# wukailu/single-stable-dreamfusion

Measured on AMD Instinct MI355X. Metric: SDS train steps/sec + rays/sec at 128×128, 1/2/4/8 MI355X, higher is better.
Workload: dtype fp16+f32; 1 GPU; C2: -O (fp16, cuda_ray, dir_text) 128x128 render, batch 1, max_steps 512, density grid update every 16 steps; global_batch=1, parallelism=dp1, backward=fused, launch=hip-graph replay, grad_exchange=none (one rank), optimizer_in_graph=True

## Files before the change

include/dfhip.h:

```cpp
#ifndef DFHIP_H
#define DFHIP_H

#include <stdint.h>

#ifdef __cplusplus
extern "C" {
#endif

typedef void *dfhip_stream_t;

enum dfhip_dtype { DFHIP_F32 = 0, DFHIP_F16 = 1, DFHIP_F64 = 2, DFHIP_BF16 = 3 };
enum dfhip_shading {
    DFHIP_SHADING_ALBEDO = 0,
    DFHIP_SHADING_TEXTURELESS = 1,
    DFHIP_SHADING_LAMBERTIAN = 2,
    DFHIP_SHADING_NORMAL = 3
};

enum dfhip_status {
    DFHIP_OK = 0,
    DFHIP_EINVAL = 1,
    DFHIP_EDTYPE = 2,
    DFHIP_ELAUNCH = 3,
    DFHIP_ENOMEM = 4
// ... 403 lines not shown
                                         const float *grad_loss, float lambda, float *loss,
                                         dfhip_stream_t stream);
int dfhip_ray_head_forward_backward_entropy_loss(
    uint32_t N, const float *ws, const float *depth, const float *image, const float *rays_d,
    const float *nears, const float *fars, const float *w1, const float *b1, const float *w2,
    const float *b2, float *out_image, float *out_depth, uint8_t *mask, const float *g_image,
    float *grad_image, float *grad_ws, float *partial, float *gw1, float *gb1, float *gw2,
    float *gb2, const float *grad_loss, float lambda, float *loss, dfhip_stream_t stream);
int dfhip_ray_head_backward_check(uint32_t N, const float *g_image, const float *ws,
                                  const float *rays_d, const float *w1, const float *b1,
                                  const float *w2, const float *b2, const float *bg_color,
                                  float *grad_image, float *grad_ws, float *grad_bg,
                                  float *partial, float *gw1, float *gb1, float *gw2, float *gb2,
                                  const float *grad_loss, float lambda, float *loss,
                                  float *found_inf, dfhip_stream_t stream);
int dfhip_ray_head_forward_backward_entropy_loss_check(
    uint32_t N, const float *ws, const float *depth, const float *image, const float *rays_d,
    const float *nears, const float *fars, const float *w1, const float *b1, const float *w2,
    const float *b2, float *out_image, float *out_depth, uint8_t *mask, const float *g_image,
    float *grad_image, float *grad_ws, float *partial, float *gw1, float *gb1, float *gw2,
    float *gb2, const float *grad_loss, float lambda, float *loss, float *found_inf,
    int defer_sum, dfhip_stream_t stream);

int dfhip_entropy_forward(uint32_t N, const float *ws, float lambda, float *loss,
                          dfhip_stream_t stream);
int dfhip_entropy_backward(uint32_t N, const float *ws, const float *grad_loss, float lambda,
                           float *grad_ws, dfhip_stream_t stream);
int dfhip_entropy_backward_accumulate(uint32_t N, const float *ws, const float *grad_loss,
                                      float lambda, float *grad_ws, dfhip_stream_t stream);

int dfhip_train_step_prologue(const float *pose, float fx, float fy, float cx, float cy,
                              uint32_t H, uint32_t W, const float *aabb, float min_near,
                              uint64_t seed, uint64_t step, int perturb, const float *alphas,
                              uint32_t min_step, uint32_t max_step, float *rays_o,
                              float *rays_d, float *nears, float *fars, float *noises,
                              float *bg_color, float *g_image, int32_t *counter,
                              dfhip_stream_t stream);
int dfhip_train_step_prologue_lr(const float *pose, float fx, float fy, float cx, float cy,
                                 uint32_t H, uint32_t W, const float *aabb, float min_near,
                                 uint64_t seed, uint64_t step, int perturb, const float *alphas,
                                 uint32_t min_step, uint32_t max_step, float *rays_o,
                                 float *rays_d, float *nears, float *fars, float *noises,
                                 float *bg_color, float *g_image, int32_t *counter,
                                 const float *lr_host, uint32_t n_lr, float *lr_dev,
                                 dfhip_stream_t stream);
int dfhip_train_step_prologue_row(const float *pose, float fx, float fy, float cx, float cy,
// ... 128 lines not shown
```

single-stable-dreamfusion_amd/_dfhip.py:

```python
from __future__ import annotations

import ctypes
import os
from pathlib import Path

import torch

LIB_PATH = Path(os.environ.get("DFHIP_LIB", Path(__file__).resolve().parent / "lib" / "libdfhip.so"))

F32, F16, F64, BF16 = 0, 1, 2, 3
_DTYPE = {torch.float32: F32, torch.float16: F16, torch.float64: F64, torch.bfloat16: BF16}

_vp, _u32, _i32, _f32 = ctypes.c_void_p, ctypes.c_uint32, ctypes.c_int, ctypes.c_float
_u64 = ctypes.c_uint64

_SIGS = {
    "dfhip_near_far_from_aabb": [_i32, _vp, _vp, _vp, _u32, _f32, _vp, _vp, _vp],
    "dfhip_get_rays": [_vp, _f32, _f32, _f32, _f32, _u32, _u32, _vp, _vp, _vp],
    "dfhip_density_grid_ema": [_vp, _vp, _u32, _u32, _f32, _vp, _vp, _vp],
    "dfhip_packbits_mean": [_vp, _u32, _vp, _f32, _vp, _vp, _vp],
    "dfhip_mean_count": [_vp, _u32, _vp, _vp],
    "dfhip_sph_from_ray": [_i32, _vp, _vp, _f32, _u32, _vp, _vp],
    "dfhip_morton3D": [_vp, _u32, _vp, _vp],
    "dfhip_morton3D_invert": [_vp, _u32, _vp, _vp],
# ... 79 lines not shown
    "dfhip_grid_field_forward_quads": [_i32, _vp, _f32, _vp, _vp, _vp, _u32, _f32, _u32, _u32,
                                       _i32, _vp, _vp, _vp, _vp, _vp, _vp, _vp, _vp, _vp, _i32,
                                       _u32, _vp, _vp],
    "dfhip_grid_field_forward_bf16": [_vp, _f32, _vp, _vp, _u32, _f32, _u32, _u32, _i32, _vp,
                                      _vp, _vp, _vp, _vp, _vp, _vp, _vp, _vp, _i32, _u32, _vp,
                                      _vp],
    "dfhip_grid_field_backward_bf16": [_vp, _vp, _f32, _vp, _vp, _vp, _vp, _vp, _vp, _vp, _vp,
                                       _i32, _u32, _vp, _vp, _vp, _u32, _vp, _vp, _vp, _vp, _vp,
                                       _vp, _i32, _vp],
    "dfhip_grid_field_backward_accumulate": [
        _vp, _vp, _f32, _vp, _vp, _vp, _vp, _vp, _vp, _vp, _vp, _i32, _u32, _vp, _vp, _vp, _u32,
        _vp, _vp, _vp, _vp, _vp, _vp, _vp, _u32, _u32, _f32, _u32, _u32, _i32, _vp, _vp, _u32,
        _vp],
    "dfhip_adam_amp_step": [_i32, _vp, _vp, _vp, _vp, _vp, _vp, _vp, _vp, _vp, _vp, _vp, _vp,
                            _vp, _vp, _f32, _f32, _i32, _vp],
    "dfhip_adam_amp_step_lr_dev": [_i32, _vp, _vp, _vp, _vp, _vp, _vp, _vp, _vp, _vp, _vp, _vp,
                                   _vp, _vp, _vp, _vp, _f32, _f32, _i32, _vp],
    "dfhip_adam_amp_step_tail": [_i32, _vp, _vp, _vp, _vp, _vp, _vp, _vp, _vp, _vp, _vp, _vp,
                                 _vp, _vp, _vp, _vp, _f32, _f32, _i32, _u32, _vp, _vp, _vp, _vp],
    "dfhip_ray_head_backward_check": [_u32, _vp, _vp, _vp, _vp, _vp, _vp, _vp, _vp, _vp, _vp,
                                      _vp, _vp, _vp, _vp, _vp, _vp, _vp, _f32, _vp, _vp, _vp],
    "dfhip_ray_head_forward_backward_entropy_loss_check": [_u32] + [_vp] * 22 + [_f32, _vp, _vp,
                                                                                 _i32, _vp],
    "dfhip_param_grad_sums": [_vp, _u32, _vp, _vp, _vp, _vp, _vp, _vp, _i32, _u32, _vp, _vp, _vp,
                              _vp, _vp, _vp, _f32, _vp, _vp, _vp],
    "dfhip_grid_field_backward_check": [_i32, _vp, _vp, _f32, _vp, _vp, _vp, _vp, _vp, _vp, _vp,
                                        _vp, _i32, _u32, _vp, _vp, _vp, _u32, _vp, _vp, _vp, _vp,
                                        _vp, _vp, _i32, _vp, _i32, _vp],
    "dfhip_march_rays_train_count_staged_quads": [_i32, _vp, _vp, _vp, _f32, _f32, _u32, _u32,
                                                  _u32, _u32, _vp, _vp, _vp, _vp, _vp, _vp, _vp,
                                                  _i32, _vp, _vp, _u32, _f32, _u32, _u32, _i32,
                                                  _u32, _vp, _vp, _vp],
    "dfhip_train_step_prologue_row": [_vp, _f32, _f32, _f32, _f32, _u32, _u32, _vp, _f32,
                                      ctypes.c_uint64, ctypes.c_uint64, _i32, _vp, _u32, _u32,
                                      _vp, _vp, _vp, _vp, _vp, _vp, _vp, _vp, _vp, _u32, _vp,
                                      _u32, _vp, _vp],
    "dfhip_ray_head_forward": [_u32, _vp, _vp, _vp, _vp, _vp, _vp, _vp, _vp, _vp, _vp, _vp, _vp,
                               _vp, _vp, _vp],
    "dfhip_ray_head_backward": [_u32, _vp, _vp, _vp, _vp, _vp, _vp, _vp, _vp, _vp, _vp, _vp, _vp,
                                _vp, _vp, _vp, _vp, _vp],
    "dfhip_ray_head_backward_entropy": [_u32, _vp, _vp, _vp, _vp, _vp, _vp, _vp, _vp, _vp, _vp,
                                        _vp, _vp, _vp, _vp, _vp, _vp, _vp, _f32, _vp],
    "dfhip_ray_head_forward_backward_entropy_loss": [_u32] + [_vp] * 22 + [_f32, _vp, _vp],
    "dfhip_ray_head_backward_entropy_loss": [_u32, _vp, _vp, _vp, _vp, _vp, _vp, _vp, _vp, _vp,
                                             _vp, _vp, _vp, _vp, _vp, _vp, _vp, _vp, _f32, _vp,
                                             _vp],
# ... 228 lines not shown
```

single-stable-dreamfusion_amd/csrc/head.hip:

```cpp
#include "common.h"
#include "field_common.h"

#include <math.h>

namespace dfhip {
namespace hd {

constexpr int kDeg = 6;
constexpr int kIn = 3 + 3 * 2 * kDeg;
constexpr int kHid = 64;
constexpr int kOut = 3;
constexpr int kW1 = kHid * kIn, kB1 = kHid, kW2 = kOut * kHid, kB2 = kOut;
constexpr int kParams = kW1 + kB1 + kW2 + kB2;
constexpr float kHalfPi = 3.141592653589793f / 2.0f;

__device__ __forceinline__ float r16(float x) { return (float)(half_t)f32_rounded(x); }

struct alignas(16) W {
    float w1t[kW1], b1[kB1], w2[kW2], b2[kB2];
};

__device__ __forceinline__ void load_w(W &w, const float *w1, const float *b1, const float *w2,
                                       const float *b2) {
    for (int i = threadIdx.x; i < kW1; i += blockDim.x) {
// ... 150 lines not shown
#pragma unroll
    for (int k = 0; k < 3; ++k) {
        g[k] = g_image[(size_t)k * N + n];
        grad_image[3 * (size_t)n + k] = g[k];
        const float bg = bg_color ? bg_color[3 * (size_t)n + k] : 1.0f;
        sw = sw + g[k] * bg;
        if (grad_bg) grad_bg[3 * (size_t)n + k] = g[k] * t;
    }
    grad_ws[n] = -sw;
}

constexpr float kLo = 1e-5f, kHi = 1.0f - 1e-5f;

__device__ __forceinline__ float entropy_grad(uint32_t N, float a, const float *g, float lambda) {
    const float scale = g[0] * lambda / (float)N;
    return (a >= kLo && a <= kHi) ? scale * (log2f(1.0f - a) - log2f(a)) : 0.0f;
}

struct FwdIO {
    const float *depth, *image, *nears, *fars;
    float *out_image, *out_depth;
    uint8_t *mask;
};

template <bool FWD>
__global__ __launch_bounds__(kThreads) void k_head_bwd_net(
    uint32_t N, const float *__restrict__ g_image , const float *__restrict__ ws,
    const float *__restrict__ rays_d, const float *w1, const float *b1, const float *w2,
    const float *b2, float *__restrict__ grad_image, float *__restrict__ grad_ws,
    float *__restrict__ partial, const float *__restrict__ ent_grad_loss, float ent_lambda,
    FwdIO io) {
    __shared__ W w;
    __shared__ alignas(16) float s_x[kRays][kIn + 1];
    __shared__ half_t s_dh[kRays][kHid];
    __shared__ half_t s_h[kRays][kHid];
    __shared__ float s_do[kRays][4];
    load_w(w, w1, b1, w2, b2);
    const int q = threadIdx.x & (kSub - 1), r = threadIdx.x / kSub;
    const uint32_t n = blockIdx.x * kRays + r;
    const bool live = n < N;
    if (live) features_part(rays_d + 3 * (size_t)n, q, s_x[r]);
    else if (q == 0)
        for (int i = 0; i < kIn; ++i) s_x[r][i] = 0.0f;
    __syncthreads();
    float x[kIn], h[kPer], o[kOut];
    load_x(s_x[r], true, x);
// ... 24 lines not shown
        grad_ws[n] = ent_grad_loss ? -sw + entropy_grad(N, ws[n], ent_grad_loss, ent_lambda)
                                   : -sw;
    }
    const float t = live ? 1.0f - ws[n] : 0.0f;
    float dout[3];
#pragma unroll
    for (int k = 0; k < 3; ++k) {
        const float dbg = r16(g[k] * t);
        dout[k] = r16(dbg * (1.0f - bg[k]) * bg[k]);
    }
#pragma unroll
    for (int jj = 0; jj < kPer; ++jj) {
        const int j = kPer * q + jj;
        float a = 0.0f;
#pragma unroll
        for (int k = 0; k < kOut; ++k) a = fmaf(dout[k], w.w2[k * kHid + j], a);
        s_dh[r][j] = (half_t)(h[jj] > 0.0f ? r16(a) : 0.0f);
        s_h[r][j] = (half_t)h[jj];
    }
    if (q == 0)
#pragma unroll
        for (int k = 0; k < kOut; ++k) s_do[r][k] = dout[k];
    __syncthreads();
    float *out = partial + (size_t)blockIdx.x * kParams;
    for (int p = threadIdx.x; p < kParams; p += blockDim.x) {
        float s = 0.0f;
        if (p < kW1) {
            const int j = p / kIn, i = p - j * kIn;
            for (int y = 0; y < kRays; ++y) s = fmaf((float)s_dh[y][j], s_x[y][i], s);
        } else if (p < kW1 + kB1) {
            const int j = p - kW1;
            for (int y = 0; y < kRays; ++y) s += (float)s_dh[y][j];
        } else if (p < kW1 + kB1 + kW2) {
            const int k = (p - kW1 - kB1) / kHid, j = (p - kW1 - kB1) - k * kHid;
            for (int y = 0; y < kRays; ++y) s = fmaf(s_do[y][k], (float)s_h[y][j], s);
        } else {
            const int k = p - kW1 - kB1 - kW2;
            for (int y = 0; y < kRays; ++y) s += s_do[y][k];
        }
        out[p] = s;
    }
}

__device__ __forceinline__ void entropy_loss_block(uint32_t N, const float *__restrict__ ws,
                                                   float lambda, float *__restrict__ loss);

__device__ __forceinline__ void wsum_block(uint32_t blk, const float *__restrict__ partial,
                                           uint32_t blocks, float *gw1, float *gb1, float *gw2,
                                           float *gb2, float *found_inf) {
    __shared__ float red[16][64];
    const int o = threadIdx.x & 63, grp = threadIdx.x >> 6;
    const int p = blk * 64 + o;
    float s = 0.0f;
    if (p < kParams) {
        uint32_t b = grp;
        for (; b + 7 * 16 < blocks; b += 8 * 16) {
            float x[8];
#pragma unroll
            for (int u = 0; u < 8; ++u) x[u] = partial[(size_t)(b + 16 * u) * kParams + p];
#pragma unroll
            for (int u = 0; u < 8; ++u) s += x[u];
        }
        for (; b < blocks; b += 16) s += partial[(size_t)b * kParams + p];
    }
    red[grp][o] = s;
// ... 281 lines not shown
    float *grad_image, float *grad_ws, float *partial, float *gw1, float *gb1, float *gw2,
    float *gb2, const float *grad_loss, float lambda, float *loss, float *found_inf,
    int defer_sum, dfhip_stream_t stream) {
    const char *name = "ray_head_forward_backward_entropy_loss_check";
    if (!loss) {
        set_error("%s: null loss", name);
        return DFHIP_EINVAL;
    }
    if (N == 0) {
        set_error("%s: N must be > 0", name);
        return DFHIP_EINVAL;
    }
    if (!w1 || !depth || !image || !nears || !fars || !out_image || !out_depth || !mask ||
        !grad_loss) {
        set_error("%s: null pointer (the combined launch needs the background network)", name);
        return DFHIP_EINVAL;
    }
    const hd::FwdIO io{depth, image, nears, fars, out_image, out_depth, mask};
    return ray_head_backward(N, g_image, ws, rays_d, w1, b1, w2, b2, nullptr, grad_image,
                             grad_ws, nullptr, partial, gw1, gb1, gw2, gb2, grad_loss, lambda,
                             stream, loss, &io, found_inf, defer_sum != 0);
}

extern "C" int dfhip_param_grad_sums(const float *mlp_partial, uint32_t mlp_parts, float *gw1,
                                     float *gb1, float *gw2, float *gb2, float *gw3, float *gb3,
                                     int accumulate, uint32_t N, const float *head_partial,
                                     float *hgw1, float *hgb1, float *hgw2, float *hgb2,
                                     const float *ws, float lambda, float *loss,
                                     float *found_inf, dfhip_stream_t stream) {
    const char *name = "param_grad_sums";
    if (!mlp_partial || mlp_parts == 0 || !gw1 || !gb1 || !gw2 || !gb2 || !gw3 || !gb3) {
        set_error("%s: null pointer or no parts in the field role", name);
        return DFHIP_EINVAL;
    }
    if (head_partial && (N == 0 || !hgw1 || !hgb1 || !hgw2 || !hgb2)) {
        set_error("%s: the head role needs N > 0 and its four gradients", name);
        return DFHIP_EINVAL;
    }
    if ((ws != nullptr) != (loss != nullptr)) {
        set_error("%s: the entropy role needs both ws and loss", name);
        return DFHIP_EINVAL;
    }
    const hd::FieldSum f{mlp_partial, mlp_parts, gw1, gb1, gw2, gb2, gw3, gb3, accumulate};
    const hd::HeadSum h{head_partial, ceil_div(N, (uint32_t)hd::kRays), hgw1, hgb1, hgw2, hgb2,
                        ws, N, lambda, loss};
    const uint32_t blocks = hd::kFieldSumBlocks + (head_partial ? hd::kHeadSumBlocks : 0u) +
// ... 40 lines not shown
```

single-stable-dreamfusion_amd/csrc/raymarching.hip:

```cpp
#include "field_common.h"
#include "march_common.h"

#include <type_traits>

namespace dfhip {
namespace rm {


template <typename T> __device__ __forceinline__ T max_value();
template <> __device__ __forceinline__ float max_value<float>() { return FLT_MAX; }
template <> __device__ __forceinline__ double max_value<double>() { return DBL_MAX; }
template <> __device__ __forceinline__ half_t max_value<half_t>() { return (half_t)65504.0f; }

template <typename scalar_t>
__global__ __launch_bounds__(256) void k_near_far(const scalar_t *__restrict__ rays_o,
                                                  const scalar_t *__restrict__ rays_d,
                                                  const scalar_t *__restrict__ aabb,
                                                  uint32_t N, float min_near,
                                                  scalar_t *nears, scalar_t *fars) {
    const uint32_t n = blockIdx.x * blockDim.x + threadIdx.x;
    if (n >= N) return;
    const Ray r = load_ray(rays_o + 3 * n, rays_d + 3 * n);
    float b[6];
#pragma unroll
// ... 280 lines not shown
    acc_t T = 1, r = 0, g = 0, b = 0, ws = 0, t = 0, d = 0;
    if (num != 0 && offset + num <= M) {
        const scalar_t *s = sigmas + offset;
        const rgb_t *c = rgbs + 3 * (size_t)offset;
        const scalar_t *dl = deltas + 2 * (size_t)offset;
        for (uint32_t i = 0; i < num; ++i) {
            const acc_t alpha = (acc_t)1.0f - (acc_t)__expf(-to_f(s[i]) * to_f(dl[2 * i]));
            const acc_t w = alpha * T;
            r = fma(w, (acc_t)to_f(c[3 * i + 0]), r);
            g = fma(w, (acc_t)to_f(c[3 * i + 1]), g);
            b = fma(w, (acc_t)to_f(c[3 * i + 2]), b);
            t += (acc_t)to_f(dl[2 * i + 1]);
            d = fma(w, t, d);
            ws += w;
            T *= (acc_t)1.0f - alpha;
            if (T < (acc_t)T_thresh) break;
        }
    }
    weights_sum[index] = (scalar_t)ws;
    depth[index] = (scalar_t)d;
    image[3 * index + 0] = (scalar_t)r;
    image[3 * index + 1] = (scalar_t)g;
    image[3 * index + 2] = (scalar_t)b;
}

template <typename scalar_t, typename rgb_t, typename acc_t>
__device__ __forceinline__ rgb_t grad_cast(acc_t v) { return (rgb_t)v; }
template <>
__device__ __forceinline__ half_t grad_cast<float, half_t, float>(float v) {
    return (half_t)f32_rounded(v);
}
template <>
__device__ __forceinline__ bf16_t grad_cast<float, bf16_t, float>(float v) {
    return (bf16_t)f32_rounded(v);
}

template <typename scalar_t, bool DENSE, typename rgb_t = scalar_t>
__global__ __launch_bounds__(64) void k_composite_train_bwd(
    const scalar_t *__restrict__ grad_ws, const scalar_t *__restrict__ grad_image,
    const scalar_t *__restrict__ sigmas, const rgb_t *__restrict__ rgbs,
    const scalar_t *__restrict__ deltas, const int32_t *__restrict__ rays,
    const scalar_t *__restrict__ weights_sum, const scalar_t *__restrict__ image,
    uint32_t M, uint32_t N, float T_thresh, scalar_t *grad_sigmas, rgb_t *grad_rgbs,
    int tail = 1) {
    typedef typename Acc<scalar_t>::type acc_t;
    const uint32_t n = blockIdx.x * 64 + threadIdx.x;
    if (n >= N) return;
    const uint32_t index = (uint32_t)rays[3 * n];
    const uint32_t offset = (uint32_t)rays[3 * n + 1];
    const uint32_t num = (uint32_t)rays[3 * n + 2];
    const scalar_t zero = (scalar_t)0.0f;
    const rgb_t czero = (rgb_t)0.0f;
    uint32_t i = 0;
    if (num != 0 && offset + num <= M) {
        const scalar_t *s = sigmas + offset;
        const rgb_t *c = rgbs + 3 * (size_t)offset;
        const scalar_t *dl = deltas + 2 * (size_t)offset;
// ... 25 lines not shown
            acc = fma(gb, fma(T, cb, -(bf - b)), acc);
            acc = fma(gw, (acc_t)1 - wsf, acc);
            gs[i] = (scalar_t)(dt * acc);
            if (T < (acc_t)T_thresh) { ++i; break; }
        }
    }
    if (DENSE) {
        const uint64_t end = min((uint64_t)offset + num, (uint64_t)M);
        for (uint64_t row = (uint64_t)offset + i; row < end; ++row) {
            grad_sigmas[row] = zero;
            grad_rgbs[3 * row] = czero; grad_rgbs[3 * row + 1] = czero; grad_rgbs[3 * row + 2] = czero;
        }
        if (tail && n == N - 1) {
            for (uint64_t row = (uint64_t)offset + num; row < M; ++row) {
                grad_sigmas[row] = zero;
                grad_rgbs[3 * row] = czero; grad_rgbs[3 * row + 1] = czero; grad_rgbs[3 * row + 2] = czero;
            }
        }
    }
}

constexpr uint32_t kCompRaysPerBlock = 16;

template <int J>
__device__ __forceinline__ float row_bcast(float v) {
    return __int_as_float(
        __builtin_amdgcn_update_dpp(0, __float_as_int(v), 0x150 + J, 0xF, 0xF, false));
}

template <typename rgb_t>
__device__ __forceinline__ void load_rgb3(const rgb_t *c, float &r, float &g, float &b) {
    r = to_f(c[0]);
    g = to_f(c[1]);
    b = to_f(c[2]);
}

struct FwdChain {
    float T = 1.0f, r = 0.0f, g = 0.0f, b = 0.0f, ws = 0.0f, t = 0.0f, d = 0.0f;
    bool alive = true;
    template <int J>
    __device__ __forceinline__ void step(float a, float om, float cr, float cg, float cb,
                                         float dl, float T_thresh) {
        const float w = alive ? row_bcast<J>(a) * T : 0.0f;
        r = fmaf(w, row_bcast<J>(cr), r);
        g = fmaf(w, row_bcast<J>(cg), g);
        b = fmaf(w, row_bcast<J>(cb), b);
        t += row_bcast<J>(dl);
        d = fmaf(w, t, d);
        ws += w;
        T *= row_bcast<J>(om);
        alive = alive && !(T < T_thresh);
    }
};

template <typename scalar_t, typename rgb_t>
__global__ __launch_bounds__(256) void k_composite_train_fwd_w(
    const scalar_t *__restrict__ sigmas, const rgb_t *__restrict__ rgbs,
    const scalar_t *__restrict__ deltas, const int32_t *__restrict__ rays, uint32_t M,
    uint32_t N, float T_thresh, scalar_t *weights_sum, scalar_t *depth, scalar_t *image) {
    const uint32_t n = blockIdx.x * kCompRaysPerBlock + (threadIdx.x >> 4);
    const int lane = (int)(threadIdx.x & 15);
    uint32_t index = 0, offset = 0, num = 0;
    if (n < N) {
        index = (uint32_t)rays[3 * n];
        offset = (uint32_t)rays[3 * n + 1];
        num = (uint32_t)rays[3 * n + 2];
        if (offset + num > M) num = 0;
    }
    FwdChain c;
    for (uint32_t base = 0; base < num && c.alive; base += 16) {
        const uint32_t cnt = min(16u, num - base);
        float a = 0.0f, om = 1.0f, cr = 0.0f, cg = 0.0f, cb = 0.0f, dl = 0.0f;
        if ((uint32_t)lane < cnt) {
            const size_t i = (size_t)offset + base + lane;
            a = 1.0f - __expf(-to_f(sigmas[i]) * to_f(deltas[2 * i]));
            om = 1.0f - a;
            dl = to_f(deltas[2 * i + 1]);
            load_rgb3(rgbs + 3 * i, cr, cg, cb);
        }
#define DFHIP_FSTEP(J) c.step<J>(a, om, cr, cg, cb, dl, T_thresh);
        DFHIP_FSTEP(0) DFHIP_FSTEP(1) DFHIP_FSTEP(2) DFHIP_FSTEP(3)
        DFHIP_FSTEP(4) DFHIP_FSTEP(5) DFHIP_FSTEP(6) DFHIP_FSTEP(7)
        DFHIP_FSTEP(8) DFHIP_FSTEP(9) DFHIP_FSTEP(10) DFHIP_FSTEP(11)
        DFHIP_FSTEP(12) DFHIP_FSTEP(13) DFHIP_FSTEP(14) DFHIP_FSTEP(15)
#undef DFHIP_FSTEP
    }
    if (lane == 0 && n < N) {
        weights_sum[index] = (scalar_t)c.ws;
        depth[index] = (scalar_t)c.d;
        image[3 * index + 0] = (scalar_t)c.r;
        image[3 * index + 1] = (scalar_t)c.g;
        image[3 * index + 2] = (scalar_t)c.b;
    }
}

struct BwdChain {
    float T = 1.0f, r = 0.0f, g = 0.0f, b = 0.0f;
    bool alive = true;
    float wl, Tl, rl, gl, bl;
    bool taken;
    template <int J>
    __device__ __forceinline__ void step(int lane, float a, float om, float cr, float cg,
                                         float cb, float T_thresh) {
        const float w = row_bcast<J>(a) * T;
        r = fmaf(w, row_bcast<J>(cr), r);
        g = fmaf(w, row_bcast<J>(cg), g);
        b = fmaf(w, row_bcast<J>(cb), b);
        T *= row_bcast<J>(om);
        const bool mine = lane == J;
        wl = mine ? w : wl;
        Tl = mine ? T : Tl;
        rl = mine ? r : rl;
        gl = mine ? g : gl;
        bl = mine ? b : bl;
        taken = mine ? alive : taken;
        alive = alive && !(T < T_thresh);
    }
};

template <typename scalar_t, bool DENSE, typename rgb_t>
__global__ __launch_bounds__(256) void k_composite_train_bwd_w(
    const scalar_t *__restrict__ grad_ws, const scalar_t *__restrict__ grad_image,
    const scalar_t *__restrict__ sigmas, const rgb_t *__restrict__ rgbs,
    const scalar_t *__restrict__ deltas, const int32_t *__restrict__ rays,
    const scalar_t *__restrict__ weights_sum, const scalar_t *__restrict__ image,
    uint32_t M, uint32_t N, float T_thresh, scalar_t *grad_sigmas, rgb_t *grad_rgbs,
    int tail) {
    const uint32_t n = blockIdx.x * kCompRaysPerBlock + (threadIdx.x >> 4);
    const int lane = (int)(threadIdx.x & 15);
    const int row_shift = (int)(threadIdx.x & 48);
    const scalar_t zero = (scalar_t)0.0f;
    const rgb_t czero = (rgb_t)0.0f;
    uint32_t index = 0, offset = 0, num = 0, num_all = 0;
    if (n < N) {
        index = (uint32_t)rays[3 * n];
        offset = (uint32_t)rays[3 * n + 1];
        num_all = (uint32_t)rays[3 * n + 2];
        num = (offset + num_all <= M) ? num_all : 0u;
    }
    uint32_t done = 0;
    if (num != 0) {
// ... 525 lines not shown
```

single-stable-dreamfusion_amd/nerf/native_step.py:

```python
import ctypes

import numpy as np
import torch

import _dfhip
import _fieldmlp
import _gridencoder
import _raymarching
from _dfhip import call, ptr, stream


SHADINGS = {"albedo": 0, "textureless": 1, "lambertian": 2}
FD_EPS = 1e-2


def eligible(trainer, shading):
    from .sd import InjectedSDS
    m, opt = trainer.model, trainer.opt
    if shading not in SHADINGS or not isinstance(trainer.guidance, InjectedSDS):
        return False
    if shading != "albedo" and not trainer.fused_backward:
        return False
    if not ((trainer.fp16 or getattr(trainer, "bf16", False)) and m.cuda_ray):
        return False
# ... 226 lines not shown
        with T("march_rays_train_emit", 24 * N, md, 52 if dirs is not None else 40):
            _raymarching.march_rays_train_emit_staged(
                self.rays_d, self.max_steps, N, cap, self.xyzs, dirs, self.deltas,
                self.rays, self.block_sums, 0, self.stage)
        if not self.quads_in_march:
            quads()
        if self.shade_code:
            with T("shading_stencil", 0, md, 12 + 84):
                call("dfhip_shading_stencil", ptr(self.xyzs), ptr(self.m_dev), cap, FD_EPS,
                     float(m.bound), ptr(self.xyz_field), ptr(self.m7), stream())
        with T("grid_field_forward", rc * hb, mf, 12 + self.L * self.C * hb + 4 + 3 * hb):
            _fieldmlp.grid_field_forward(self.xyz_field, m.bound, self.table,
                                         self.encoder.offsets, S, Hb, gridtype, align, self.mlp,
                                         self.enc, self.sigma_field, self.albedo, self.m_field,
                                         quads=self.quads)
        rgb = self.albedo
        if self.shade_code:
            with T("shading_forward", 0, md, 28 + 3 * hb + 12 + 4 + 3 * hb + 12):
                call(self._shade_fwd, ptr(self.sigma_field), ptr(self.albedo),
                     ptr(self.dirs), ptr(self.light), self.ratio, FD_EPS, self.shade_code,
                     ptr(self.m_dev), cap, ptr(self.sigma), ptr(self.color), ptr(self.normal),
                     ptr(self.orient_partial), self.lam_orient, ptr(self.orient), None, stream())
            rgb = self.color
        with T("composite_rays_train_forward", 32 * N, md, 4 + 3 * hb + 8):
            _raymarching.composite_rays_train_forward_mixed(
                self.sigma, rgb, self.deltas, self.rays, cap, N, 1e-4, self.ws, self.depth,
                self.image)
        bw = self._bg_weights()
        combined = (not self.two_pass and self.lam > 0 and bw[0] is not None
                    and bool(getattr(self.trainer, "combined_head", True)))
        fi = self.found_inf
        defer = combined and self.merged_sums
        if not combined:
            with T("ray_head_forward", 60 * N):
                call("dfhip_ray_head_forward", N, ptr(self.ws), ptr(self.depth), ptr(self.image),
                     ptr(self.rays_d), ptr(self.nears), ptr(self.fars), *[ptr(w) for w in bw],
                     ptr(self.bg_color), ptr(self.out_image), ptr(self.out_depth),
                     ptr(self.mask), stream())
        if self.two_pass:
            if self.lam > 0:
                call("dfhip_entropy_forward", N, ptr(self.ws), self.lam, ptr(self.loss),
                     stream())
            self._add_orient_loss()
            self._backward_two_pass(bw, scale)
            return self.loss
        gbw = self._bg_grads()
        head_args = (N, ptr(self.g_image), ptr(self.ws), ptr(self.rays_d), *[ptr(w) for w in bw],
                     ptr(self.bg_color), ptr(self.grad_image), ptr(self.grad_ws), None,
                     ptr(self.head_partial), *[ptr(g) for g in gbw])
        with T("ray_head_backward", 60 * N if not combined else 120 * N):
            if combined and (fi is not None or defer):
                call("dfhip_ray_head_forward_backward_entropy_loss_check", N, ptr(self.ws),
                     ptr(self.depth), ptr(self.image), ptr(self.rays_d), ptr(self.nears),
                     ptr(self.fars), *[ptr(w) for w in bw], ptr(self.out_image),
                     ptr(self.out_depth), ptr(self.mask), ptr(self.g_image), ptr(self.grad_image),
# ... 8 lines not shown
                     ptr(scale), self.lam, ptr(self.loss), stream())
            elif fi is not None and bw[0] is not None:
                call("dfhip_ray_head_backward_check", *head_args,
                     ptr(scale) if self.lam > 0 else None, self.lam,
                     ptr(self.loss) if self.lam > 0 else None, ptr(fi), stream())
            elif self.lam > 0:
                call("dfhip_ray_head_backward_entropy_loss", *head_args, ptr(scale), self.lam,
                     ptr(self.loss), stream())
            else:
                call("dfhip_ray_head_backward", *head_args, stream())
        self._add_orient_loss()
        with T("composite_rays_train_backward", 44 * N, md, 4 + 3 * hb + 8 + 4 + 3 * hb):
            _raymarching.composite_rays_train_backward_mixed(
                self.grad_ws, self.grad_image, self.sigma, rgb, self.deltas, self.rays,
                self.ws, self.image, cap, N, 1e-4, self.grad_sigma,
                self.grad_color if self.shade_code else self.grad_albedo, False)
        if self.shade_code:
            with T("shading_backward", 0, md, 28 + 3 * hb + 12 + 4 + 3 * hb + 28 + 21 * hb):
                call(self._shade_bwd, ptr(self.sigma_field), ptr(self.albedo),
                     ptr(self.dirs), ptr(self.light), self.ratio, FD_EPS, self.shade_code,
                     ptr(self.m_dev), cap, ptr(self.grad_sigma), ptr(self.grad_color),
                     ptr(scale), self.lam_orient, ptr(self.grad_sigma_field),
                     ptr(self.grad_albedo), stream())
        from gridencoder.grid import _parts
        per_bwd = 2 * self.L * self.C * hb + 4 + 3 * hb + 12
        with T("field_mlp_backward", 4 * _fieldmlp.params_count(), mf, per_bwd):
            _fieldmlp.grid_field_backward(
                self.enc, self.xyz_field, m.bound, self.mlp, self.grad_sigma_field,
                self.grad_albedo, self.d_enc, self.mlp_partial, [p.grad for p in self.mlp],
                self.encoder.offsets, self.rows, S, Hb, gridtype, align, None, None,
                _parts(self.rows, self.C), self.m_field, found_inf=fi,
                defer_sum=self.merged_sums)
            if self.merged_sums:
                call("dfhip_param_grad_sums", ptr(self.mlp_partial),
                     _fieldmlp.backward_parts(self.fcap) if self.fcap else 1,
                     *[ptr(p.grad) for p in self.mlp], 0, N,
                     ptr(self.head_partial) if defer else None,
                     *[ptr(g) if defer else None for g in gbw],
                     ptr(self.ws) if defer else None, self.lam,
                     ptr(self.loss) if defer else None, ptr(fi), stream())
        return self.loss

    def _backward_two_pass(self, bw, scale):
        m = self.trainer.model
        N, cap = self.N, self.cap
        S, Hb, gridtype, align, _ = self.meta
        from gridencoder.grid import _parts
# ... 130 lines not shown
```

single-stable-dreamfusion_amd/nerf/utils.py:

```python
import glob
import math
import os
import random
import time

import numpy as np
import torch
import torch.distributed as dist
import torch.nn as nn
import torch.nn.functional as F


def custom_meshgrid(*args):
    return torch.meshgrid(*args, indexing="ij")


def safe_normalize(x, eps=1e-20):
    return x / torch.sqrt(torch.clamp(torch.sum(x * x, -1, keepdim=True), min=eps))


@torch.autocast("cuda", enabled=False)
def get_rays(poses, intrinsics, H, W, N=-1, error_map=None):
    device = poses.device
    B = poses.shape[0]
# ... 198 lines not shown
        self.amp_dtype = torch.bfloat16 if self.bf16 else torch.float16
        self.best_mode = best_mode
        self.use_loss_as_metric = use_loss_as_metric
        self.report_metric_at_train = report_metric_at_train
        self.max_keep_ckpt = max_keep_ckpt
        self.eval_interval = eval_interval
        self.use_checkpoint = use_checkpoint
        self.use_tensorboardX = use_tensorboardX
        self.time_stamp = time.strftime("%Y-%m-%d_%H-%M-%S")
        self.scheduler_update_every_step = scheduler_update_every_step
        self.fused_backward = fused_backward
        self.graph_step = graph_step
        self.dp_in_graph = None
        self._graphs = {}
        self.native_optimizer = True
        self.native_step = True
        self.stencil_bin = True
        self.kept_clean_scratch = True
        self.combined_head = True
        self.fold_overflow_check = True
        self.merged_grad_sums = True
        self.store_live_count = True
        self.quads_in_march = True
        self.module_buckets = True
        self.native_losses = True
        self._native_opt = None
        self.step_hook = None
        self.device = device if device is not None else torch.device(
            f"cuda:{local_rank}" if torch.cuda.is_available() else "cpu")

        model.to(self.device)
        self.model = model
        if world_size > 1 and dist.is_available() and dist.is_initialized():
            with torch.no_grad():
                for t in list(model.parameters()) + list(model.buffers()):
                    dist.broadcast(t.data, src=0)
        self._capture_stream = None
        if (self.device.type == "cuda" and dist.is_available() and dist.is_initialized()
                and dist.get_backend() == "nccl"):
            self._capture_stream = torch.cuda.Stream(device=self.device)
            self._capture_stream.wait_stream(torch.cuda.current_stream())
            with torch.cuda.stream(self._capture_stream):
                dist.all_reduce(torch.zeros(1, device=self.device))
            torch.cuda.current_stream().wait_stream(self._capture_stream)
        if getattr(model, "cuda_ray", False) and self.device.type == "cuda":
            model.grid_generator = torch.Generator(device=self.device).manual_seed(
# ... 415 lines not shown
```

Before: 17.60 million rays/s.

## Fuse composite forward, background head and composite backward into one ray-chain kernel

Adds a single kernel that composites rays forward, runs the background MLP head forward and backward with the entropy gradient, and computes per-sample sigma and rgb gradients. These steps were previously separate launches. The fusion removes several kernel launches and the global round-trips for ws, image, grad_ws and grad_image between them. The cost is that one block does serial per-ray marching plus MLP work, which may reduce occupancy through extra shared memory and registers. It also recomputes sample loads for the backward chain. The DPP broadcast helper switches from update_dpp to mov_dpp.

Result: faster. 17.81 million rays/s (median of 6 runs) (+1.2%).

```diff
diff --git a/include/dfhip.h b/include/dfhip.h
--- a/include/dfhip.h
+++ b/include/dfhip.h
@@ -449,6 +449,16 @@
     float *gb2, const float *grad_loss, float lambda, float *loss, float *found_inf,
     int defer_sum, dfhip_stream_t stream);
 
+int dfhip_ray_chain_train(
+    int rgb_dtype, const float *sigmas, const void *rgbs, const float *deltas,
+    const int32_t *rays, uint32_t M, uint32_t N, float T_thresh, float *ws, float *depth,
+    float *image, const float *rays_d, const float *nears, const float *fars, const float *w1,
+    const float *b1, const float *w2, const float *b2, float *out_image, float *out_depth,
+    uint8_t *mask, const float *g_image, float *grad_image, float *grad_ws, float *partial,
+    float *gw1, float *gb1, float *gw2, float *gb2, const float *grad_loss, float lambda,
+    float *loss, float *found_inf, int defer_sum, float *grad_sigmas, void *grad_rgbs,
+    dfhip_stream_t stream);
+
 int dfhip_entropy_forward(uint32_t N, const float *ws, float lambda, float *loss,
                           dfhip_stream_t stream);
 int dfhip_entropy_backward(uint32_t N, const float *ws, const float *grad_loss, float lambda,
diff --git a/single-stable-dreamfusion_amd/_dfhip.py b/single-stable-dreamfusion_amd/_dfhip.py
--- a/single-stable-dreamfusion_amd/_dfhip.py
+++ b/single-stable-dreamfusion_amd/_dfhip.py
@@ -125,6 +125,8 @@
                                       _vp, _vp, _vp, _vp, _vp, _vp, _vp, _f32, _vp, _vp, _vp],
     "dfhip_ray_head_forward_backward_entropy_loss_check": [_u32] + [_vp] * 22 + [_f32, _vp, _vp,
                                                                                  _i32, _vp],
+    "dfhip_ray_chain_train": [_i32] + [_vp] * 4 + [_u32, _u32, _f32] + [_vp] * 22 + [
+        _f32, _vp, _vp, _i32, _vp, _vp, _vp],
     "dfhip_param_grad_sums": [_vp, _u32, _vp, _vp, _vp, _vp, _vp, _vp, _i32, _u32, _vp, _vp, _vp,
                               _vp, _vp, _vp, _f32, _vp, _vp, _vp],
     "dfhip_grid_field_backward_check": [_i32, _vp, _vp, _f32, _vp, _vp, _vp, _vp, _vp, _vp, _vp,
diff --git a/single-stable-dreamfusion_amd/csrc/chain_common.h b/single-stable-dreamfusion_amd/csrc/chain_common.h
--- /dev/null
+++ b/single-stable-dreamfusion_amd/csrc/chain_common.h
@@ -0,0 +1,75 @@
+#pragma once
+
+#include "common.h"
+
+namespace dfhip {
+namespace rm {
+
+template <typename scalar_t, typename rgb_t, typename acc_t>
+__device__ __forceinline__ rgb_t grad_cast(acc_t v) { return (rgb_t)v; }
+template <>
+__device__ __forceinline__ half_t grad_cast<float, half_t, float>(float v) {
+    return (half_t)f32_rounded(v);
+}
+template <>
+__device__ __forceinline__ bf16_t grad_cast<float, bf16_t, float>(float v) {
+    return (bf16_t)f32_rounded(v);
+}
+
+template <int J>
+__device__ __forceinline__ float row_bcast(float v) {
+    return __int_as_float(__builtin_amdgcn_mov_dpp(__float_as_int(v), 0x150 + J, 0xF, 0xF, true));
+}
+
+template <typename rgb_t>
+__device__ __forceinline__ void load_rgb3(const rgb_t *c, float &r, float &g, float &b) {
+    r = to_f(c[0]);
+    g = to_f(c[1]);
+    b = to_f(c[2]);
+}
+
+struct FwdChain {
+    float T = 1.0f, r = 0.0f, g = 0.0f, b = 0.0f, ws = 0.0f, t = 0.0f, d = 0.0f;
+    bool alive = true;
+    template <int J>
+    __device__ __forceinline__ void step(float a, float om, float cr, float cg, float cb,
+                                         float dl, float T_thresh) {
+        const float aT = row_bcast<J>(a) * T;
+        const float w = alive ? aT : 0.0f;
+        r = fmaf(w, row_bcast<J>(cr), r);
+        g = fmaf(w, row_bcast<J>(cg), g);
+        b = fmaf(w, row_bcast<J>(cb), b);
+        t += row_bcast<J>(dl);
+        d = fmaf(w, t, d);
+        ws += w;
+        T *= row_bcast<J>(om);
+        alive = alive && !(T < T_thresh);
+    }
+};
+
+struct BwdChain {
+    float T = 1.0f, r = 0.0f, g = 0.0f, b = 0.0f;
+    bool alive = true;
+    float wl, Tl, rl, gl, bl;
+    bool taken;
+    template <int J>
+    __device__ __forceinline__ void step(int lane, float a, float om, float cr, float cg,
+                                         float cb, float T_thresh) {
+        const float w = row_bcast<J>(a) * T;
+        r = fmaf(w, row_bcast<J>(cr), r);
+        g = fmaf(w, row_bcast<J>(cg), g);
+        b = fmaf(w, row_bcast<J>(cb), b);
+        T *= row_bcast<J>(om);
+        const bool mine = lane == J;
+        wl = mine ? w : wl;
+        Tl = mine ? T : Tl;
+        rl = mine ? r : rl;
+        gl = mine ? g : gl;
+        bl = mine ? b : bl;
+        taken = mine ? alive : taken;
+        alive = alive && !(T < T_thresh);
+    }
+};
+
+}
+}
diff --git a/single-stable-dreamfusion_amd/csrc/head.hip b/single-stable-dreamfusion_amd/csrc/head.hip
--- a/single-stable-dreamfusion_amd/csrc/head.hip
+++ b/single-stable-dreamfusion_amd/csrc/head.hip
@@ -1,4 +1,5 @@
 #include "common.h"
+#include "chain_common.h"
 #include "field_common.h"
 
 #include <math.h>
@@ -196,6 +197,12 @@
     float *out_image, *out_depth;
     uint8_t *mask;
 };
+
+__device__ __forceinline__ void write_partials(const float (&s_x)[kRays][kIn + 1],
+                                               const half_t (&s_dh)[kRays][kHid],
+                                               const half_t (&s_h)[kRays][kHid],
+                                               const float (&s_do)[kRays][4],
+                                               float *__restrict__ partial);
 
 template <bool FWD>
 __global__ __launch_bounds__(kThreads) void k_head_bwd_net(
@@ -266,6 +273,14 @@
 #pragma unroll
         for (int k = 0; k < kOut; ++k) s_do[r][k] = dout[k];
     __syncthreads();
+    write_partials(s_x, s_dh, s_h, s_do, partial);
+}
+
+__device__ __forceinline__ void write_partials(const float (&s_x)[kRays][kIn + 1],
+                                               const half_t (&s_dh)[kRays][kHid],
+                                               const half_t (&s_h)[kRays][kHid],
+                                               const float (&s_do)[kRays][4],
+                                               float *__restrict__ partial) {
     float *out = partial + (size_t)blockIdx.x * kParams;
     for (int p = threadIdx.x; p < kParams; p += blockDim.x) {
         float s = 0.0f;
@@ -285,6 +300,207 @@
         out[p] = s;
     }
 }
+
+struct RayChainArgs {
+    const float *sigmas;
+    const void *rgbs;
+    const float *deltas;
+    const int32_t *rays;
+    uint32_t M, N;
+    float T_thresh;
+    float *ws, *depth, *image;
+    const float *rays_d, *nears, *fars, *w1, *b1, *w2, *b2;
+    float *out_image, *out_depth;
+    uint8_t *mask;
+    const float *g_image;
+    float *grad_image, *grad_ws, *partial;
+    const float *ent_grad_loss;
+    float ent_lambda;
+    float *grad_sigmas;
+    void *grad_rgbs;
+};
+
+template <typename rgb_t> struct RawWin {
+    float sg = 0.0f, dt = 0.0f, dl = 0.0f;
+    rgb_t c0 = (rgb_t)0.0f, c1 = (rgb_t)0.0f, c2 = (rgb_t)0.0f;
+    bool in = false;
+};
+
+template <typename rgb_t>
+__device__ __forceinline__ RawWin<rgb_t> load_win(const RayChainArgs &p, uint32_t offset,
+                                                  uint32_t num, uint32_t base, int lane) {
+    RawWin<rgb_t> v;
+    v.in = base < num && (uint32_t)lane < num - base;
+    if (v.in) {
+        const size_t i = (size_t)offset + base + lane;
+        const rgb_t *c = (const rgb_t *)p.rgbs + 3 * i;
+        v.sg = p.sigmas[i];
+        v.dt = p.deltas[2 * i];
+        v.dl = p.deltas[2 * i + 1];
+        v.c0 = c[0];
+        v.c1 = c[1];
+        v.c2 = c[2];
+    }
+    return v;
+}
+
+struct WinOps {
+    float a, om, cr, cg, cb;
+};
+template <typename rgb_t> __device__ __forceinline__ WinOps win_ops(const RawWin<rgb_t> &v) {
+    WinOps o;
+    o.a = v.in ? 1.0f - __expf(-v.sg * v.dt) : 0.0f;
+    o.om = 1.0f - o.a;
+    o.cr = to_f(v.c0);
+    o.cg = to_f(v.c1);
+    o.cb = to_f(v.c2);
+    return o;
+}
+
+#define DFHIP_16(STEP)                                                                      \
+    STEP(0) STEP(1) STEP(2) STEP(3) STEP(4) STEP(5) STEP(6) STEP(7) STEP(8) STEP(9) STEP(10) \
+    STEP(11) STEP(12) STEP(13) STEP(14) STEP(15)
+
+template <typename rgb_t>
+__global__ __launch_bounds__(kThreads) void k_ray_chain(RayChainArgs p) {
+    __shared__ W w;
+    __shared__ alignas(16) float s_x[kRays][kIn + 1];
+    __shared__ half_t s_dh[kRays][kHid];
+    __shared__ half_t s_h[kRays][kHid];
+    __shared__ float s_do[kRays][4];
+    const int q = threadIdx.x & (kSub - 1), r = threadIdx.x / kSub;
+    const int row_shift = (int)(threadIdx.x & 48);
+    const uint32_t N = p.N;
+    const uint32_t n = blockIdx.x * kRays + r;
+    const bool live = n < N;
+    const float T_thresh = p.T_thresh;
+    rgb_t *grad_rgbs = (rgb_t *)p.grad_rgbs;
+
+    uint32_t offset = 0, num = 0, num_all = 0;
+    float d[3] = {0.0f, 0.0f, 0.0f}, g[3] = {0.0f, 0.0f, 0.0f}, nr = 0.0f, fr = 0.0f;
+    if (live) {
+        offset = (uint32_t)p.rays[3 * n + 1];
+        num_all = (uint32_t)p.rays[3 * n + 2];
+        num = (offset + num_all <= p.M) ? num_all : 0u;
+#pragma unroll
+        for (int c = 0; c < 3; ++c) d[c] = p.rays_d[3 * (size_t)n + c];
+#pragma unroll
+        for (int k = 0; k < 3; ++k) g[k] = p.g_image[(size_t)k * N + n];
+        nr = p.nears[n];
+        fr = p.fars[n];
+    }
+    RawWin<rgb_t> cur = load_win<rgb_t>(p, offset, num, 0, q);
+
+    load_w(w, p.w1, p.b1, p.w2, p.b2);
+    if (live) features_part(d, q, s_x[r]);
+    else if (q == 0)
+        for (int i = 0; i < kIn; ++i) s_x[r][i] = 0.0f;
+    __syncthreads();
+
+    rm::FwdChain c;
+    for (uint32_t base = 0; base < num && c.alive; base += 16) {
+        if (base != 0) cur = load_win<rgb_t>(p, offset, num, base, q);
+        const WinOps v = win_ops(cur);
+        const float dl = cur.dl;
+#define DFHIP_FSTEP(J) c.step<J>(v.a, v.om, v.cr, v.cg, v.cb, dl, T_thresh);
+        DFHIP_16(DFHIP_FSTEP)
+#undef DFHIP_FSTEP
+    }
+    const float wsv = c.ws, rf = c.r, gf = c.g, bf = c.b;
+    if (q == 0 && live) {
+        p.ws[n] = wsv;
+        p.depth[n] = c.d;
+        p.image[3 * (size_t)n + 0] = rf;
+        p.image[3 * (size_t)n + 1] = gf;
+        p.image[3 * (size_t)n + 2] = bf;
+    }
+
+    float bg[3], dout[3], gw;
+    {
+        float x[kIn], h[kPer], o[kOut];
+        load_x(s_x[r], true, x);
+        mlp_part(w, x, q, h, o);
+#pragma unroll
+        for (int k = 0; k < 3; ++k) bg[k] = sigmoid16(o[k]);
+        float sw = 0.0f;
+#pragma unroll
+        for (int k = 0; k < 3; ++k) sw = sw + g[k] * bg[k];
+        gw = -sw + entropy_grad(N, wsv, p.ent_grad_loss, p.ent_lambda);
+        if (live && q == 0) {
+            const float t = 1.0f - wsv;
+#pragma unroll
+            for (int k = 0; k < 3; ++k) {
+                const float img = k == 0 ? rf : (k == 1 ? gf : bf);
+                p.out_image[(size_t)k * N + n] = img + t * bg[k];
+                p.grad_image[3 * (size_t)n + k] = g[k];
+            }
+            const float dd = c.d - nr;
+            p.out_depth[n] = (dd < 0.0f ? 0.0f : dd) / (fr - nr);
+            p.mask[n] = nr < fr ? 1 : 0;
+            p.grad_ws[n] = gw;
+        }
+        const float t = live ? 1.0f - wsv : 0.0f;
+#pragma unroll
+        for (int k = 0; k < 3; ++k) {
+            const float dbg = r16(g[k] * t);
+            dout[k] = r16(dbg * (1.0f - bg[k]) * bg[k]);
+        }
+#pragma unroll
+        for (int jj = 0; jj < kPer; ++jj) {
+            const int j = kPer * q + jj;
+            float a = 0.0f;
+#pragma unroll
+            for (int k = 0; k < kOut; ++k) a = fmaf(dout[k], w.w2[k * kHid + j], a);
+            s_dh[r][j] = (half_t)(h[jj] > 0.0f ? r16(a) : 0.0f);
+            s_h[r][j] = (half_t)h[jj];
+        }
+        if (q == 0)
+#pragma unroll
+            for (int k = 0; k < kOut; ++k) s_do[r][k] = dout[k];
+    }
+
+    const float gr = g[0], gg = g[1], gb = g[2];
+#define DFHIP_SAMPLE_GRAD(I, WL, TL, RL, GL, BL, DT, CR, CG, CB)                              \
+    {                                                                                         \
+        grad_rgbs[3 * (I) + 0] = rm::grad_cast<float, rgb_t>(gr * (WL));                      \
+        grad_rgbs[3 * (I) + 1] = rm::grad_cast<float, rgb_t>(gg * (WL));                      \
+        grad_rgbs[3 * (I) + 2] = rm::grad_cast<float, rgb_t>(gb * (WL));                      \
+        float acc = fmaf(gr, fmaf((TL), (CR), -(rf - (RL))), gg * fmaf((TL), (CG), -(gf - (GL)))); \
+        acc = fmaf(gb, fmaf((TL), (CB), -(bf - (BL))), acc);                                  \
+        acc = fmaf(gw, 1.0f - wsv, acc);                                                      \
+        p.grad_sigmas[(I)] = (DT) * acc;                                                      \
+    }
+    uint32_t done = 0;
+    rm::BwdChain b;
+    for (uint32_t base = 0; base < num && b.alive; base += 16) {
+        cur = load_win<rgb_t>(p, offset, num, base, q);
+        const WinOps v = win_ops(cur);
+        b.wl = b.Tl = b.rl = b.gl = b.bl = 0.0f;
+        b.taken = false;
+#define DFHIP_BSTEP(J) b.step<J>(q, v.a, v.om, v.cr, v.cg, v.cb, T_thresh);
+        DFHIP_16(DFHIP_BSTEP)
+#undef DFHIP_BSTEP
+        const bool taken = b.taken && cur.in;
+        if (taken) {
+            const size_t i = (size_t)offset + base + q;
+            DFHIP_SAMPLE_GRAD(i, b.wl, b.Tl, b.rl, b.gl, b.bl, cur.dt, v.cr, v.cg, v.cb)
+        }
+        done = base + (uint32_t)__popcll((__ballot(taken) >> row_shift) & 0xFFFFull);
+    }
+#undef DFHIP_SAMPLE_GRAD
+    if (live) {
+        const uint64_t end = min((uint64_t)offset + num_all, (uint64_t)p.M);
+        for (uint64_t row = (uint64_t)offset + done + q; row < end; row += 16) {
+            p.grad_sigmas[row] = 0.0f;
+            grad_rgbs[3 * row] = (rgb_t)0.0f;
+            grad_rgbs[3 * row + 1] = (rgb_t)0.0f;
+            grad_rgbs[3 * row + 2] = (rgb_t)0.0f;
+        }
+    }
+    __syncthreads();
+    write_partials(s_x, s_dh, s_h, s_do, p.partial);
+}
+#undef DFHIP_16
 
 __device__ __forceinline__ void entropy_loss_block(uint32_t N, const float *__restrict__ ws,
                                                    float lambda, float *__restrict__ loss);
@@ -612,6 +828,46 @@
                              stream, loss, &io, found_inf, defer_sum != 0);
 }
 
+extern "C" int dfhip_ray_chain_train(
+    int rgb_dtype, const float *sigmas, const void *rgbs, const float *deltas,
+    const int32_t *rays, uint32_t M, uint32_t N, float T_thresh, float *ws, float *depth,
+    float *image, const float *rays_d, const float *nears, const float *fars, const float *w1,
+    const float *b1, const float *w2, const float *b2, float *out_image, float *out_depth,
+    uint8_t *mask, const float *g_image, float *grad_image, float *grad_ws, float *partial,
+    float *gw1, float *gb1, float *gw2, float *gb2, const float *grad_loss, float lambda,
+    float *loss, float *found_inf, int defer_sum, float *grad_sigmas, void *grad_rgbs,
+    dfhip_stream_t stream) {
+    const char *name = "ray_chain_train";
+    if (N == 0) {
+        set_error("%s: N must be > 0", name);
+        return DFHIP_EINVAL;
+    }
+    if (!sigmas || !rgbs || !deltas || !rays || !ws || !depth || !image || !rays_d || !nears ||
+        !fars || !w1 || !b1 || !w2 || !b2 || !out_image || !out_depth || !mask || !g_image ||
+        !grad_image || !grad_ws || !partial || !gw1 || !gb1 || !gw2 || !gb2 || !grad_loss ||
+        !loss || !grad_sigmas || !grad_rgbs) {
+        set_error("%s: null pointer (only found_inf may be null)", name);
+        return DFHIP_EINVAL;
+    }
+    const hd::RayChainArgs a{sigmas, rgbs, deltas, rays, M, N, T_thresh, ws, depth, image,
+                             rays_d, nears, fars, w1, b1, w2, b2, out_image, out_depth, mask,
+                             g_image, grad_image, grad_ws, partial, grad_loss, lambda,
+                             grad_sigmas, grad_rgbs};
+    hipStream_t s = as_stream(stream);
+    const uint32_t blocks = ceil_div(N, (uint32_t)hd::kRays);
+    if (rgb_dtype == DFHIP_F32) hd::k_ray_chain<float><<<blocks, hd::kThreads, 0, s>>>(a);
+    else if (rgb_dtype == DFHIP_F16) hd::k_ray_chain<half_t><<<blocks, hd::kThreads, 0, s>>>(a);
+    else if (rgb_dtype == DFHIP_BF16) hd::k_ray_chain<bf16_t><<<blocks, hd::kThreads, 0, s>>>(a);
+    else {
+        set_error("%s: rgb dtype must be f32, f16 or bf16 (got %d)", name, rgb_dtype);
+        return DFHIP_EDTYPE;
+    }
+    if (!defer_sum)
+        hd::k_head_wsum<<<ceil_div((uint32_t)hd::kParams, 64u) + 1u, 1024, 0, s>>>(
+            partial, blocks, gw1, gb1, gw2, gb2, ws, N, lambda, loss, found_inf);
+    return check_launch(name);
+}
+
 extern "C" int dfhip_param_grad_sums(const float *mlp_partial, uint32_t mlp_parts, float *gw1,
                                      float *gb1, float *gw2, float *gb2, float *gw3, float *gb3,
                                      int accumulate, uint32_t N, const float *head_partial,
diff --git a/single-stable-dreamfusion_amd/csrc/raymarching.hip b/single-stable-dreamfusion_amd/csrc/raymarching.hip
--- a/single-stable-dreamfusion_amd/csrc/raymarching.hip
+++ b/single-stable-dreamfusion_amd/csrc/raymarching.hip
@@ -1,5 +1,6 @@
 #include "field_common.h"
 #include "march_common.h"
+#include "chain_common.h"
 
 #include <type_traits>
 
@@ -326,17 +327,6 @@
     image[3 * index + 0] = (scalar_t)r;
     image[3 * index + 1] = (scalar_t)g;
     image[3 * index + 2] = (scalar_t)b;
-}
-
-template <typename scalar_t, typename rgb_t, typename acc_t>
-__device__ __forceinline__ rgb_t grad_cast(acc_t v) { return (rgb_t)v; }
-template <>
-__device__ __forceinline__ half_t grad_cast<float, half_t, float>(float v) {
-    return (half_t)f32_rounded(v);
-}
-template <>
-__device__ __forceinline__ bf16_t grad_cast<float, bf16_t, float>(float v) {
-    return (bf16_t)f32_rounded(v);
 }
 
 template <typename scalar_t, bool DENSE, typename rgb_t = scalar_t>
@@ -408,37 +398,6 @@
 
 constexpr uint32_t kCompRaysPerBlock = 16;
 
-template <int J>
-__device__ __forceinline__ float row_bcast(float v) {
-    return __int_as_float(
-        __builtin_amdgcn_update_dpp(0, __float_as_int(v), 0x150 + J, 0xF, 0xF, false));
-}
-
-template <typename rgb_t>
-__device__ __forceinline__ void load_rgb3(const rgb_t *c, float &r, float &g, float &b) {
-    r = to_f(c[0]);
-    g = to_f(c[1]);
-    b = to_f(c[2]);
-}
-
-struct FwdChain {
-    float T = 1.0f, r = 0.0f, g = 0.0f, b = 0.0f, ws = 0.0f, t = 0.0f, d = 0.0f;
-    bool alive = true;
-    template <int J>
-    __device__ __forceinline__ void step(float a, float om, float cr, float cg, float cb,
-                                         float dl, float T_thresh) {
-        const float w = alive ? row_bcast<J>(a) * T : 0.0f;
-        r = fmaf(w, row_bcast<J>(cr), r);
-        g = fmaf(w, row_bcast<J>(cg), g);
-        b = fmaf(w, row_bcast<J>(cb), b);
-        t += row_bcast<J>(dl);
-        d = fmaf(w, t, d);
-        ws += w;
-        T *= row_bcast<J>(om);
-        alive = alive && !(T < T_thresh);
-    }
-};
-
 template <typename scalar_t, typename rgb_t>
 __global__ __launch_bounds__(256) void k_composite_train_fwd_w(
     const scalar_t *__restrict__ sigmas, const rgb_t *__restrict__ rgbs,
@@ -479,30 +438,6 @@
         image[3 * index + 2] = (scalar_t)c.b;
     }
 }
-
-struct BwdChain {
-    float T = 1.0f, r = 0.0f, g = 0.0f, b = 0.0f;
-    bool alive = true;
-    float wl, Tl, rl, gl, bl;
-    bool taken;
-    template <int J>
-    __device__ __forceinline__ void step(int lane, float a, float om, float cr, float cg,
-                                         float cb, float T_thresh) {
-        const float w = row_bcast<J>(a) * T;
-        r = fmaf(w, row_bcast<J>(cr), r);
-        g = fmaf(w, row_bcast<J>(cg), g);
-        b = fmaf(w, row_bcast<J>(cb), b);
-        T *= row_bcast<J>(om);
-        const bool mine = lane == J;
-        wl = mine ? w : wl;
-        Tl = mine ? T : Tl;
-        rl = mine ? r : rl;
-        gl = mine ? g : gl;
-        bl = mine ? b : bl;
-        taken = mine ? alive : taken;
-        alive = alive && !(T < T_thresh);
-    }
-};
 
 template <typename scalar_t, bool DENSE, typename rgb_t>
 __global__ __launch_bounds__(256) void k_composite_train_bwd_w(
diff --git a/single-stable-dreamfusion_amd/nerf/native_step.py b/single-stable-dreamfusion_amd/nerf/native_step.py
--- a/single-stable-dreamfusion_amd/nerf/native_step.py
+++ b/single-stable-dreamfusion_amd/nerf/native_step.py
@@ -272,15 +272,29 @@
                      ptr(self.m_dev), cap, ptr(self.sigma), ptr(self.color), ptr(self.normal),
                      ptr(self.orient_partial), self.lam_orient, ptr(self.orient), None, stream())
             rgb = self.color
-        with T("composite_rays_train_forward", 32 * N, md, 4 + 3 * hb + 8):
-            _raymarching.composite_rays_train_forward_mixed(
-                self.sigma, rgb, self.deltas, self.rays, cap, N, 1e-4, self.ws, self.depth,
-                self.image)
         bw = self._bg_weights()
         combined = (not self.two_pass and self.lam > 0 and bw[0] is not None
                     and bool(getattr(self.trainer, "combined_head", True)))
         fi = self.found_inf
         defer = combined and self.merged_sums
+        chain = defer and bool(getattr(self.trainer, "fused_ray_chain", True))
+        self.ray_chain = chain
+        if chain:
+            with T("ray_chain", (32 + 120 + 44) * N, md,
+                   (4 + 3 * hb + 8) + (4 + 3 * hb + 8 + 4 + 3 * hb)):
+                call("dfhip_ray_chain_train", _dfhip._DTYPE[rgb.dtype], ptr(self.sigma), ptr(rgb),
+                     ptr(self.deltas), ptr(self.rays), cap, N, 1e-4, ptr(self.ws),
+                     ptr(self.depth), ptr(self.image), ptr(self.rays_d), ptr(self.nears),
+                     ptr(self.fars), *[ptr(w) for w in bw], ptr(self.out_image),
+                     ptr(self.out_depth), ptr(self.mask), ptr(self.g_image),
+                     ptr(self.grad_image), ptr(self.grad_ws), ptr(self.head_partial),
+                     *[ptr(g) for g in self._bg_grads()], ptr(scale), self.lam, ptr(self.loss),
+                     ptr(fi), 1, ptr(self.grad_sigma), ptr(self.grad_albedo), stream())
+            return self._field_backward(fi, defer, hb)
+        with T("composite_rays_train_forward", 32 * N, md, 4 + 3 * hb + 8):
+            _raymarching.composite_rays_train_forward_mixed(
+                self.sigma, rgb, self.deltas, self.rays, cap, N, 1e-4, self.ws, self.depth,
+                self.image)
         if not combined:
             with T("ray_head_forward", 60 * N):
                 call("dfhip_ray_head_forward", N, ptr(self.ws), ptr(self.depth), ptr(self.image),
@@ -335,7 +349,13 @@
                      ptr(self.m_dev), cap, ptr(self.grad_sigma), ptr(self.grad_color),
                      ptr(scale), self.lam_orient, ptr(self.grad_sigma_field),
                      ptr(self.grad_albedo), stream())
+        return self._field_backward(fi, defer, hb)
+
+    def _field_backward(self, fi, defer, hb):
         from gridencoder.grid import _parts
+        m, N, T, mf = self.trainer.model, self.N, _dfhip.timed, self.m_field
+        S, Hb, gridtype, align, _ = self.meta
+        gbw = self._bg_grads()
         per_bwd = 2 * self.L * self.C * hb + 4 + 3 * hb + 12
         with T("field_mlp_backward", 4 * _fieldmlp.params_count(), mf, per_bwd):
             _fieldmlp.grid_field_backward(
diff --git a/single-stable-dreamfusion_amd/nerf/utils.py b/single-stable-dreamfusion_amd/nerf/utils.py
--- a/single-stable-dreamfusion_amd/nerf/utils.py
+++ b/single-stable-dreamfusion_amd/nerf/utils.py
@@ -244,6 +244,7 @@
         self.merged_grad_sums = True
         self.store_live_count = True
         self.quads_in_march = True
+        self.fused_ray_chain = True
         self.module_buckets = True
         self.native_losses = True
         self._native_opt = None
```
